# foollh/PicoPose

Measured on AMD Instinct MI355X. Metric: image-crops/sec (224x224, 162 templates), higher is better.
Workload: dtype f32 tensors; networks: f32 operands split into 2 f16 terms (22 bits) on f16 MFMA with f32 accumulate; stage-1 contraction: f16 MFMA operands, f32 accumulate, exact f32 re-evaluation of near-ties; PnP f64

## Files before the change

include/picopose_hip.h:

```cpp
#ifndef PICOPOSE_HIP_H
#define PICOPOSE_HIP_H

#include <stddef.h>
#include <stdint.h>

#ifdef __cplusplus
extern "C" {
#endif

#define PP_OK 0
#define PP_EINVAL (-1)
#define PP_EWORKSPACE (-2)
#define PP_ELAUNCH (-3)

#define PP_MATCH_EXACT 0
#define PP_MATCH_FAST 1

const char* pp_strerror(int code);
int pp_version(void);

int pp_prof_enable(int max_records);
int pp_prof_collect(float* out_ms, int max_out, int* count);
int pp_prof_gemm_enable(int max_records);
int pp_prof_gemm_collect(double* ms, double* flops, int* launches);
// ... 125 lines not shown
int pp_sum_slices(const float* part, int S, int M, int N, const float* bias, int act, float* out, void* stream);
int pp_hl_patch_columns(const float* x, int ld_x, int c, long long rows, void* hl, int ld_h, int col0, void* stream);

int pp_split_weights_t(const float* w, long long n, int terms, void* out, float* scale, void* stream);
int pp_split_activation_t(const float* x, long long batch_stride, int B, int P, int row_stride, int C, int relu, void* out,
                          int ld_h, int terms, void* stream);
int pp_hl_patch_columns_t(const float* x, int ld_x, int c, long long rows, void* out, int ld_h, int col0, int terms, void* stream);
int pp_layernorm_t(const float* x, const float* gamma, const float* beta, int rows, int C, float eps, float* y, void* out, int terms,
                   void* stream);
int pp_resize_bilinear_nhwc_t(const float* in, int B, int H, int W, int C, int Ho, int Wo, float mul, void* out, int terms,
                              void* stream);
int pp_resize_bilinear_nhwc_dual(const float* in, int B, int H, int W, int C, int Ho, int Wo, float mul, float* out, void* out_operand,
                                 int terms, void* stream);
int pp_warp_nhwc_t(const float* feat, int feat_batch, const float* flow, int B, int H, int W, int C, int ld_flow, void* out,
                   int ld_h, int terms, void* stream);
int pp_attention_t(const void* qkv_operand, int terms, int B, int T, int heads, int head_dim, float scale, float* out,
                   void* out_operand, void* stream);

int pp_attention(const float* qkv, int B, int T, int heads, int head_dim, float scale, float* out, void* stream);
int pp_attention_split(const float* qkv, int B, int T, int heads, int head_dim, float scale, float* out, void* out_hl,
                       void* stream);
int pp_attention_ex(const float* qkv, int B, int T, int heads, int head_dim, float scale, int prec, float* out, void* out_hl,
                    void* stream);
int pp_attention_hl(const void* qkv_hl, int B, int T, int heads, int head_dim, float scale, float* out, void* out_hl,
                    void* stream);
int pp_attention_train(const float* qkv, int B, int T, int heads, int head_dim, float scale, float* out, float* lse2, void* stream);
int pp_attention_backward(const float* qkv, const float* out, const float* dout, const float* lse2, const float* gpair, int B, int T,
                          int heads, int head_dim, float scale, float* Dws, float* dqkv, void* stream);

int pp_layernorm(const float* x, const float* gamma, const float* beta, int rows, int C, float eps,
                 float* y, void* stream);
int pp_layernorm_split(const float* x, const float* gamma, const float* beta, int rows, int C, float eps, float* y,
                       void* hl, void* stream);
int pp_softmax_rows(float* x, int rows, int n, int ld, void* stream);
int pp_groupnorm_nhwc(const float* x, const float* gamma, const float* beta, int B, int HW, int C,
                      int groups, float eps, int relu, float* y, void* stream);
int pp_transpose_batched(const float* in, long long in_batch_stride, int B, int R, int C, float* out,
                         long long out_batch_stride, int ld_out, int col_off, void* stream);
int pp_assemble_tokens(const float* patches, const float* cls_token, const float* pos, int B, int T, int C,
                       float* tokens, void* stream);
int pp_normalize_rows(const float* x, int rows, int n, float eps, float* y, void* stream);

int pp_resize_bilinear_nhwc(const float* in, int B, int H, int W, int C, int Ho, int Wo, float mul,
                            float* out, void* stream);
int pp_resize_bilinear_nhwc_hl(const float* in, int B, int H, int W, int C, int Ho, int Wo, float mul, void* out_hl,
                               void* stream);
int pp_warp_nhwc(const float* feat, int feat_batch, const float* flow, int B, int H, int W, int C, int ld_flow,
                 float* out, int ld_out, void* stream);
int pp_warp_nhwc_hl(const float* feat, int feat_batch, const float* flow, int B, int H, int W, int C, int ld_flow,
                    void* out_hl, int ld_h, void* stream);
int pp_avgpool2_nhwc(const float* in, int B, int H, int W, int C, float* out, void* stream);
int pp_gather_rows(const float* src, const long long* index, long long n_src_rows, long long row_floats, int n, float* dst,
                   void* stream);

int pp_crop_resize_normalize(const unsigned char* image, int H, int W, const unsigned char* mask, int y1, int y2, int x1,
                             int x2, int S, int rgb_mask_flag, const double* mean3, const double* std3, float* out_rgb,
                             float* out_mask, void* stream);
int pp_depth_points_nearest(const float* depth_m, int H, int W, int y1, int y2, int x1, int x2, int P, float fx, float fy,
                            float cx, float cy, float* out_pts, void* stream);
int pp_corr_lookup_nhwc(const float* f1, int ld_f1, const float* f2_l0, const float* f2_l1, const float* f2_l2,
                        int f2_batch, const float* flow, int B, int H, int W, int C, int levels, int radius,
                        int ld_flow, float* out, int ld_out, void* stream);
int pp_corr_lookup_nhwc_ex(const float* f1, int ld_f1, const float* f2_l0, const float* f2_l1, const float* f2_l2,
                           int f2_batch, const float* flow, int B, int H, int W, int C, int levels, int radius,
                           int ld_flow, int prec, float* out, int ld_out, void* stream);

int pp_conv_narrow_hl(const void* x_hl, int ld_x, int B, int H, int W, int C, const float* weight, const float* bias, int ksize,
                      int n_out, const float* residual, float* out, void* stream);
int pp_conv_narrow_f32(const float* x, int ld_x, int B, int H, int W, int C, const float* weight, const float* bias, int ksize,
                       int n_out, const float* residual, float* out, void* stream);

int pp_winograd_input_f32(const float* x, int ld_x, long long batch_stride, int B, int H, int W, int C, int relu, float* U, void* stream);
int pp_winograd_weight_f32(const float* w, int Cout, int Cin, int ldw, float* V, void* stream);
int pp_winograd_output_f32(const float* Y, int B, int H, int W, int Cout, const float* bias, int act, const float* residual,
                           const float* residual2, float* out, int ldc, void* stream);

int pp_winograd4_input_hl(const void* x_hl, int ld_x, long long batch_stride, int B, int H, int W, int C, int relu, void* U_hl, long long P_pad,
                          void* stream);
int pp_winograd4_weight_f32(const float* w, int Cout, int Cin, int ldw, float* V, void* stream);
int pp_winograd4_output(const float* Y, int ld_y, int B, int H, int W, int Cout, const float* bias, int act, const float* residual,
                        const float* residual2, float* out, int ldc, void* out_hl, int ld_h, int c_relu, long long P_pad, void* stream);

int pp_winograd4_chain(const float* Y, int ld_y, int B, int H, int W, int C, const float* bias, int act, int c_relu, void* U_hl, long long P_pad,
                       void* stream);

int pp_winograd_chain_f32(const float* Y, int B, int H, int W, int C, const float* bias, int act, int relu_next, float* U, void* stream);

int pp_set_saturation_word(unsigned int* word);

int pp_saturation_take(unsigned int* word, unsigned int* slot, void* stream);


int pp_corr_lookup_nhwc_hl(const void* f1_hl, int ld_f1, const void* f2_hl_l0, const void* f2_hl_l1, const void* f2_hl_l2,
                           int f2_batch, const float* flow, int B, int H, int W, int C, int levels, int radius, int ld_flow,
                           float* out, int ld_out, void* stream);

int pp_pnp_ransac(const float* tar_pts_2d, const float* src_pts_3d, const float* K, const float* tem_pose,
                  const int64_t* tar_pts, const int64_t* src_pts, int P, int H, int W, int N, int iterations,
                  float reproj_threshold, double* rot, double* tvec, double* inlier_ratio, int32_t* success,
                  int32_t* num_points, void* stream);

int pp_pnp_ransac_debug(const float* tar_pts_2d, const float* src_pts_3d, const float* K, const float* tem_pose,
                        const int64_t* tar_pts, const int64_t* src_pts, int P, int H, int W, int N, int iterations,
                        float reproj_threshold, double* rot, double* tvec, double* inlier_ratio, int32_t* success,
                        int32_t* num_points, double* refit_branches, void* stream);

// ... 240 lines not shown
```

picopose_amd/_lib.py:

```python
import ctypes
import os
import re

from .build import LIB

_HEADER = os.path.join(os.path.dirname(os.path.abspath(__file__)), "..", "include", "picopose_hip.h")

PP_OK = 0
PP_MATCH_EXACT = 0
PP_MATCH_FAST = 1
PP_BANK_F32 = 0
PP_BANK_F16 = 1

_lib = None


class PpGemmDesc(ctypes.Structure):
    _fields_ = [
        ("A", ctypes.c_void_p), ("B", ctypes.c_void_p), ("C", ctypes.c_void_p), ("bias", ctypes.c_void_p),
        ("gamma", ctypes.c_void_p), ("residual", ctypes.c_void_p), ("residual2", ctypes.c_void_p),
        ("M", ctypes.c_int), ("N", ctypes.c_int), ("K", ctypes.c_int),
        ("lda", ctypes.c_int), ("ldb", ctypes.c_int), ("ldc", ctypes.c_int), ("b_kn", ctypes.c_int),
        ("batch0", ctypes.c_int), ("batch1", ctypes.c_int),
        ("a_bs0", ctypes.c_longlong), ("a_bs1", ctypes.c_longlong), ("b_bs0", ctypes.c_longlong),
# ... 73 lines not shown
                                              vp, vp]
        L.pp_similarity_volume.argtypes = [vp, vp, vp, i32, i32, i32, i32, vp, vp]
        L.pp_calc_pred_Ms.argtypes = [vp, vp, vp, vp, vp, vp, i32, f32, vp, vp]
        L.pp_pose_recovery_2d.argtypes = [vp, vp, vp, vp, vp, vp, i32, vp, vp]
        L.pp_init_correspondences.argtypes = [vp, vp, i32, i32, i32, vp, vp, vp]
        L.pp_stage3_correspondences.argtypes = [vp, vp, i32, i32, i32, f32, vp, vp, vp]
        L.pp_gather_valid.argtypes = [vp, vp, i32, i32, i32, i32, i32, vp, vp, vp]
        L.pp_gemm.argtypes = [c.POINTER(PpGemmDesc), vp]
        L.pp_split_f16x3.argtypes = [vp, c.c_longlong, vp, vp, vp]
        L.pp_split_activation.argtypes = [vp, c.c_longlong, i32, i32, i32, i32, i32, vp, vp]
        L.pp_split_activation_ld.argtypes = [vp, c.c_longlong, i32, i32, i32, i32, i32, vp, i32, vp]
        L.pp_conv_narrow_hl.argtypes = [vp, i32, i32, i32, i32, i32, vp, vp, i32, i32, vp, vp, vp]
        L.pp_conv_narrow_f32.argtypes = [vp, i32, i32, i32, i32, i32, vp, vp, i32, i32, vp, vp, vp]
        L.pp_winograd_input_f32.argtypes = [vp, i32, c.c_longlong, i32, i32, i32, i32, i32, vp, vp]
        L.pp_winograd_weight_f32.argtypes = [vp, i32, i32, i32, vp, vp]
        L.pp_winograd_output_f32.argtypes = [vp, i32, i32, i32, i32, vp, i32, vp, vp, vp, i32, vp]
        L.pp_winograd4_input_hl.argtypes = [vp, i32, c.c_longlong, i32, i32, i32, i32, i32, vp, c.c_longlong, vp]
        L.pp_winograd4_weight_f32.argtypes = [vp, i32, i32, i32, vp, vp]
        L.pp_winograd4_output.argtypes = [vp, i32, i32, i32, i32, i32, vp, i32, vp, vp, vp, i32, vp, i32, i32, c.c_longlong, vp]
        L.pp_winograd4_chain.argtypes = [vp, i32, i32, i32, i32, i32, vp, i32, i32, vp, c.c_longlong, vp]
        L.pp_winograd_chain_f32.argtypes = [vp, i32, i32, i32, i32, vp, i32, i32, vp, vp]
        L.pp_set_saturation_word.argtypes = [vp]
        L.pp_saturation_take.argtypes = [vp, vp, vp]
        L.pp_split_weights_t.argtypes = [vp, c.c_longlong, i32, vp, vp, vp]
        L.pp_split_weights_ws.argtypes = [vp, c.c_longlong, i32, vp, vp, vp, vp]
        L.pp_split_activation_t.argtypes = [vp, c.c_longlong, i32, i32, i32, i32, i32, vp, i32, i32, vp]
        L.pp_hl_patch_columns_t.argtypes = [vp, i32, i32, c.c_longlong, vp, i32, i32, i32, vp]
        L.pp_layernorm_t.argtypes = [vp, vp, vp, i32, i32, f32, vp, vp, i32, vp]
        L.pp_resize_bilinear_nhwc_t.argtypes = [vp, i32, i32, i32, i32, i32, i32, f32, vp, i32, vp]
        L.pp_resize_bilinear_nhwc_dual.argtypes = [vp, i32, i32, i32, i32, i32, i32, f32, vp, vp, i32, vp]
        L.pp_warp_nhwc_t.argtypes = [vp, i32, vp, i32, i32, i32, i32, i32, vp, i32, i32, vp]
        L.pp_attention_t.argtypes = [vp, i32, i32, i32, i32, i32, f32, vp, vp, vp]
        L.pp_sum_slices.argtypes = [vp, i32, i32, i32, vp, i32, vp, vp]
        L.pp_hl_patch_columns.argtypes = [vp, i32, i32, c.c_longlong, vp, i32, i32, vp]
        L.pp_warp_nhwc_hl.argtypes = [vp, i32, vp, i32, i32, i32, i32, i32, vp, i32, vp]
        L.pp_attention.argtypes = [vp, i32, i32, i32, i32, f32, vp, vp]
        L.pp_attention_split.argtypes = [vp, i32, i32, i32, i32, f32, vp, vp, vp]
        L.pp_attention_ex.argtypes = [vp, i32, i32, i32, i32, f32, i32, vp, vp, vp]
        L.pp_attention_hl.argtypes = [vp, i32, i32, i32, i32, f32, vp, vp, vp]
        L.pp_attention_train.argtypes = [vp, i32, i32, i32, i32, f32, vp, vp, vp]
        L.pp_attention_backward.argtypes = [vp, vp, vp, vp, vp, i32, i32, i32, i32, f32, vp, vp, vp]
        L.pp_layernorm.argtypes = [vp, vp, vp, i32, i32, f32, vp, vp]
        L.pp_layernorm_split.argtypes = [vp, vp, vp, i32, i32, f32, vp, vp, vp]
        L.pp_softmax_rows.argtypes = [vp, i32, i32, i32, vp]
        L.pp_groupnorm_nhwc.argtypes = [vp, vp, vp, i32, i32, i32, i32, f32, i32, vp, vp]
        L.pp_transpose_batched.argtypes = [vp, c.c_longlong, i32, i32, i32, vp, c.c_longlong, i32, i32, vp]
        L.pp_assemble_tokens.argtypes = [vp, vp, vp, i32, i32, i32, vp, vp]
        L.pp_normalize_rows.argtypes = [vp, i32, i32, f32, vp, vp]
        L.pp_resize_bilinear_nhwc.argtypes = [vp, i32, i32, i32, i32, i32, i32, f32, vp, vp]
        L.pp_resize_bilinear_nhwc_hl.argtypes = [vp, i32, i32, i32, i32, i32, i32, f32, vp, vp]
        L.pp_warp_nhwc.argtypes = [vp, i32, vp, i32, i32, i32, i32, i32, vp, i32, vp]
        L.pp_avgpool2_nhwc.argtypes = [vp, i32, i32, i32, i32, vp, vp]
        L.pp_gather_rows.argtypes = [vp, vp, c.c_longlong, c.c_longlong, i32, vp, vp]
        L.pp_depth_points_nearest.argtypes = [vp, i32, i32, i32, i32, i32, i32, i32, f32, f32, f32, f32, vp, vp]
        L.pp_crop_resize_normalize.argtypes = [vp, i32, i32, vp, i32, i32, i32, i32, i32, i32, c.POINTER(c.c_double),
                                               c.POINTER(c.c_double), vp, vp, vp]
        L.pp_corr_lookup_nhwc.argtypes = [vp, i32, vp, vp, vp, i32, vp, i32, i32, i32, i32, i32, i32, i32, vp, i32, vp]
        L.pp_corr_lookup_nhwc_ex.argtypes = [vp, i32, vp, vp, vp, i32, vp, i32, i32, i32, i32, i32, i32, i32, i32, vp, i32, vp]
        L.pp_corr_lookup_nhwc_hl.argtypes = [vp, i32, vp, vp, vp, i32, vp, i32, i32, i32, i32, i32, i32, i32, vp, i32, vp]
        L.pp_pnp_ransac.argtypes = [vp, vp, vp, vp, vp, vp, i32, i32, i32, i32, i32, f32, vp, vp, vp, vp, vp, vp]
        L.pp_pnp_ransac_debug.argtypes = [vp, vp, vp, vp, vp, vp, i32, i32, i32, i32, i32, f32, vp, vp, vp, vp, vp, vp, vp]
        L.pp_pnp_ransac_refine.argtypes = [vp, vp, vp, vp, vp, vp, i32, i32, i32, i32, i32, f32, i32, c.c_double] + [vp] * 10
        L.pp_pnp_refine_lm.argtypes = [vp] * 6 + [i32, i32, i32, c.c_double] + [vp] * 6
        L.pp_rgbd_ransac.argtypes = [vp] * 6 + [i32] * 4 + [vp, i32, i32, i32, vp, vp, i32] + [vp] * 9
        L.pp_train_keypoints_workspace_bytes.restype = sz
        L.pp_train_keypoints_workspace_bytes.argtypes = [i32]
        L.pp_train_keypoints.argtypes = [vp, vp, i32, i32, vp, vp, i32, i32] + [vp] * 10 + [i32, vp, vp, vp, sz, vp]
        L.pp_batchnorm_train_workspace_bytes.restype = sz
        L.pp_batchnorm_train_workspace_bytes.argtypes = [i32, i32]
        L.pp_batchnorm_train.argtypes = [vp, vp, vp, i32, i32, f32, f32, vp, vp, i32, vp, vp, vp, vp, sz, vp]
        L.pp_gather_normalize_rows.argtypes = [vp, c.c_longlong, vp, i32, i32, f32, vp, vp]
        L.pp_xent_diag_rows.argtypes = [vp, i32, i32, f32, vp, vp]
        L.pp_flow_loss_blocks.argtypes = []
        L.pp_flow_loss_sums.argtypes = [vp, vp, vp, i32, i32, i32, f32, vp, vp]
        ll = c.c_longlong
        L.pp_colsum_workspace_bytes.restype = sz
        L.pp_colsum_workspace_bytes.argtypes = [ll, i32]
        L.pp_colsum.argtypes = [vp, ll, i32, i32, vp, vp, sz, vp]
        L.pp_act_forward.argtypes = [vp, ll, i32, vp, vp]
        L.pp_act_backward.argtypes = [vp, vp, ll, i32, vp, vp]
        L.pp_elementwise.argtypes = [i32, vp, vp, ll, i32, vp, vp]
        L.pp_layernorm_backward.argtypes = [vp, vp, vp, i32, i32, f32, vp, vp, vp]
        L.pp_groupnorm_backward_nhwc.argtypes = [vp, vp, vp, vp, i32, i32, i32, i32, f32, i32, vp, vp, vp, vp]
        L.pp_softmax_backward_rows.argtypes = [vp, vp, ll, i32, vp, vp]
        L.pp_xent_diag_backward.argtypes = [vp, i32, i32, f32, vp, vp, vp]
        L.pp_normalize_rows_backward.argtypes = [vp, ll, vp, vp, i32, i32, f32, vp, vp]
        L.pp_scatter_add_rows.argtypes = [vp, vp, i32, i32, vp, vp]
        L.pp_im2col_nhwc.argtypes = [vp, i32, i32, i32, i32, i32, i32, i32, vp, vp]
        L.pp_col2im_nhwc.argtypes = [vp, i32, i32, i32, i32, i32, i32, i32, vp, vp]
        L.pp_simvol_backward.argtypes = [vp, vp, vp, i32, i32, i32, vp, vp]
        L.pp_im2col_t_nhwc.argtypes = [vp, i32, i32, i32, i32, i32, i32, i32, vp, vp]
        L.pp_pow2_scale.argtypes = [vp, ll, vp, vp]
        L.pp_pow2_scale_ws.argtypes = [vp, ll, vp, vp, vp]
        L.pp_split_scaled_t.argtypes = [vp, ll, i32, i32, vp, vp, i32, vp]
        L.pp_split_transpose_t.argtypes = [vp, ll, i32, i32, vp, vp, i32, vp]
        L.pp_split_transpose_ld.argtypes = [vp, ll, i32, i32, vp, vp, ll, i32, vp]
        L.pp_im2col_t_operand.argtypes = [vp, i32, i32, i32, i32, i32, i32, i32, vp, i32, vp]
        L.pp_split_with_scale_t.argtypes = [vp, ll, i32, vp, vp, vp]
        L.pp_batchnorm_train_backward_workspace_bytes.restype = sz
        L.pp_batchnorm_train_backward_workspace_bytes.argtypes = [ll, i32]
        L.pp_batchnorm_train_backward.argtypes = [vp, vp, vp, vp, ll, i32, f32, i32, vp, vp, vp, vp, sz, vp]
        L.pp_resize_bilinear_backward_nhwc.argtypes = [vp, i32, i32, i32, i32, i32, i32, f32, vp, vp]
        L.pp_avgpool2_backward_nhwc.argtypes = [vp, i32, i32, i32, i32, i32, vp, vp]
        L.pp_warp_backward_nhwc.argtypes = [vp, vp, vp, i32, i32, i32, i32, i32, vp, vp, vp]
        L.pp_corr_lookup_backward_nhwc.argtypes = [vp, vp, vp, vp, i32, i32, i32, i32, i32, i32, i32, i32, vp, vp, vp, vp]
        L.pp_warp_backward_nhwc_fixed.argtypes = [vp, vp, vp, i32, i32, i32, i32, i32, vp, vp, vp]
# ... 67 lines not shown
```

picopose_amd/csrc/pp_sample.hip:

```cpp

#include <hip/hip_runtime.h>
#include <stdlib.h>
#include <stdint.h>
#include "../../include/picopose_hip.h"
#include "pp_common.h"
#include "pp_crop_dev.h"

namespace {

typedef float f4 __attribute__((ext_vector_type(4)));

__device__ __forceinline__ float resize_blend(float a, float b, float c, float d, float hx, float lx, float hy, float ly, float mul) {
#pragma clang fp contract(off)
    const float top = fmaf(hx, a, lx * b), bot = fmaf(hx, c, lx * d);
    return (hy * top + ly * bot) * mul;
}

__global__ __launch_bounds__(256) void resize_kernel(const float* __restrict__ in, int H, int W, int C,
                                                     int Ho, int Wo, float mul, float* __restrict__ out,
                                                     _Float16* __restrict__ out_hl, int terms) {
    const int b = blockIdx.z, oy = blockIdx.y, tid = threadIdx.x;
    const float sy = Ho > 1 ? (float)(H - 1) / (float)(Ho - 1) : 0.f;
    const float sx = Wo > 1 ? (float)(W - 1) / (float)(Wo - 1) : 0.f;
    const float fy = sy * (float)oy;
// ... 379 lines not shown
                }
            };
            load_chunk(0, ra0, rb0);
            if (nk > 1) load_chunk(1, ra1, rb1);
            for (int kc = 0; kc < nk; kc += 2) {
                chunk(kc, ra0, rb0);
                if (kc + 1 < nk) chunk(kc + 1, ra1, rb1);
            }
            __syncthreads();
#pragma unroll
            for (int i = 0; i < 2; ++i)
#pragma unroll
                for (int j = 0; j < 2; ++j)
#pragma unroll
                    for (int e = 0; e < 16; ++e)
                        S[(i * 32 + (e >> 2) * 8 + lh * 4 + (e & 3)) * CSP + wv * 64 + j * 32 + l31] =
                            acc[i][j][e] * (EXACT ? inv_sqrt_c : inv_sqrt_c / (PP_A_SCALE * PP_A_SCALE));
            __syncthreads();
            for (int idx = tid; idx < CM * win * win; idx += 256) {
                const int m = idx / (win * win), o = idx - m * (win * win), ai = o / win, bi = o - ai * win;
                const int dx = s_bx[m] - ox, dy = s_by[m] - oy;
                if (s_state[m] == 0 && dx >= 0 && dx <= fit && dy >= 0 && dy <= fit) {
                    const float cx = s_cx[m], cy = s_cy[m];
                    const float wx1 = cx - floorf(cx), wy1 = cy - floorf(cy), wx0 = 1.f - wx1, wy0 = 1.f - wy1;
                    const float* t = S + m * CSP + (dy + bi) * CRW + dx + ai;
                    out[((size_t)b * H * W + (size_t)(y0 + (m >> 3)) * W + x0 + (m & 7)) * ld_out + l * win * win + o] =
                        t[0] * (wx0 * wy0) + t[1] * (wx1 * wy0) + t[CRW] * (wx0 * wy1) + t[CRW + 1] * (wx1 * wy1);
                }
            }
            __syncthreads();
            if (tid < CM && s_state[tid] == 0) {
                const int dx = s_bx[tid] - ox, dy = s_by[tid] - oy;
                if (dx >= 0 && dx <= fit && dy >= 0 && dy <= fit) {
                    s_state[tid] = 1;
                    atomicSub(&s_todo, 1);
                }
            }
            __syncthreads();
        }
        __syncthreads();
    }
}

__global__ __launch_bounds__(256) void gather_rows_kernel(const float* __restrict__ src, const long long* __restrict__ index,
                                                          long long row, long long nsrc, float* __restrict__ dst) {
    const long long r = index[blockIdx.y];
    if (r < 0 || r >= nsrc) return;
    const f4* s4 = (const f4*)(src + r * row);
    f4* d4 = (f4*)(dst + (long long)blockIdx.y * row);
    const long long n4 = row >> 2;
    for (long long i = (long long)blockIdx.x * 256 + threadIdx.x; i < n4; i += (long long)gridDim.x * 256) d4[i] = s4[i];
}

__global__ __launch_bounds__(64) void saturation_take_kernel(unsigned* __restrict__ word, unsigned* __restrict__ slot) {
    if (threadIdx.x == 0) *slot = atomicExch(word, 0u);
}

__global__ __launch_bounds__(256) void crop_resize_kernel(const unsigned char* __restrict__ img, int W,
                                                          const unsigned char* __restrict__ mask, int y1, int y2, int x1,
                                                          int x2, int S, int mask_rgb, double m0, double m1, double m2,
                                                          double s0, double s1, double s2, float* __restrict__ out_rgb,
                                                          float* __restrict__ out_mask) {
    const int i = blockIdx.x * 256 + threadIdx.x;
    if (i >= S * S) return;
    const int oy = i / S, ox = i - oy * S, h = y2 - y1, w = x2 - x1;
    int ya, yb, xa, xb;
    double fy, fx;
    pp_crop_taps(oy, h, S, ya, yb, fy);
    pp_crop_taps(ox, w, S, xa, xb, fx);
    const double mean[3] = {m0, m1, m2}, stdv[3] = {s0, s1, s2};
    auto px = [&](int yy, int xx, int c) -> double {
        const size_t p = (size_t)(y1 + yy) * W + (x1 + xx);
        double v = (double)img[p * 3 + (2 - c)] / 255.0;
        if (mask_rgb && mask && mask[p] == 0) v = 0.0;
        return v;
    };
#pragma unroll
    for (int c = 0; c < 3; ++c) out_rgb[(size_t)c * S * S + i] = pp_crop_blend(px, c, ya, yb, xa, xb, fx, fy, mean[c], stdv[c]);
    if (out_mask) {
        const int yi = pp_crop_nearest(oy, h, S), xi = pp_crop_nearest(ox, w, S);
        out_mask[i] = mask ? (float)mask[(size_t)(y1 + yi) * W + (x1 + xi)] : 1.f;
    }
}

__global__ __launch_bounds__(256) void depth_points_kernel(const float* __restrict__ depth, int W, int y1, int y2, int x1,
                                                           int x2, int P, float fx, float fy, float cx, float cy,
                                                           float* __restrict__ out) {
    const int i = blockIdx.x * 256 + threadIdx.x;
    if (i >= P * P) return;
    const int oy = i / P, ox = i - oy * P, h = y2 - y1, w = x2 - x1;
    const int y = y1 + pp_crop_nearest(oy, h, P), x = x1 + pp_crop_nearest(ox, w, P);
    pp_depth_point(depth[(size_t)y * W + x], x, y, fx, fy, cx, cy, out + 3 * i);
}


constexpr int NRW_PITCH = 144;

template <int KS, int NOUT, bool F32IN = false>
__global__ __launch_bounds__(256) void conv_narrow_kernel(const _Float16* __restrict__ x, int ldx, int H, int W, int C,
                                                          const float* __restrict__ w, const float* __restrict__ bias,
                                                          const float* __restrict__ residual, float* __restrict__ out) {
    constexpr int R = KS / 2;
    extern __shared__ __attribute__((aligned(16))) unsigned char nsm[];
    const int TH = 256 / W, bands = H / TH;
    const int b = blockIdx.x / bands, y0 = (blockIdx.x % bands) * TH;
    const int tid = threadIdx.x, ty = tid / W, tx = tid % W;
// ... 204 lines not shown
    if (ld_f1 < C || ld_f1 % 4 != 0 || ((uintptr_t)f1 % 16) != 0 || f2_batch <= 0) return PP_EINVAL;
    if (levels < 1 || levels > MAXL || radius < 1 || radius > MAXR) return PP_EINVAL;
    if ((levels > 1 && !f2_l1) || (levels > 2 && !f2_l2)) return PP_EINVAL;
    if ((H >> (levels - 1)) < 1 || (W >> (levels - 1)) < 1 || ld_flow < 2) return PP_EINVAL;
    const int win = 2 * radius + 1;
    if (ld_out < levels * win * win) return PP_EINVAL;
    const char* te = getenv("PP_CORR_TILED");
    const bool tiled = !(te && te[0] == '0');
    const bool aligned = (((uintptr_t)f2_l0 | (levels > 1 ? (uintptr_t)f2_l1 : 0) | (levels > 2 ? (uintptr_t)f2_l2 : 0)) % 16) == 0;
    if (tiled && H % CT == 0 && W % CT == 0 && C % CK == 0 && aligned)
        return corr_tiled_launch(false, f1, ld_f1, f2_l0, f2_l1, f2_l2, f2_batch, flow, B, H, W, C, levels, radius, ld_flow, out, ld_out, stream,
                                 prec == PP_PREC_F32, prec == PP_PREC_F16);
    const size_t smem = (size_t)4 * (C + MAXL * TW * TW) * sizeof(float);
    hipLaunchKernelGGL(corr_lookup_kernel, dim3((H * W + 3) / 4, B), dim3(256), smem, (hipStream_t)stream, f1, ld_f1,
                       f2_batch, f2_l0, f2_l1, f2_l2, flow, H, W, C, levels, radius, ld_flow, 1.0f / sqrtf((float)C), out,
                       ld_out);
    return pp_last_launch();
}

int pp_corr_lookup_nhwc_hl(const void* f1_hl, int ld_f1, const void* f2_hl_l0, const void* f2_hl_l1, const void* f2_hl_l2,
                           int f2_batch, const float* flow, int B, int H, int W, int C, int levels, int radius, int ld_flow,
                           float* out, int ld_out, void* stream) {
    if (!f1_hl || !f2_hl_l0 || !flow || !out || B <= 0 || H <= 0 || W <= 0 || C <= 0 || f2_batch <= 0) return PP_EINVAL;
    if (H % CT != 0 || W % CT != 0 || C % CK != 0 || ld_f1 < C || ld_f1 % 8 != 0) return PP_EINVAL;
    if (((uintptr_t)f1_hl | (uintptr_t)f2_hl_l0 | (uintptr_t)f2_hl_l1 | (uintptr_t)f2_hl_l2) % 16 != 0) return PP_EINVAL;
    if (levels < 1 || levels > MAXL || radius < 1 || radius > MAXR) return PP_EINVAL;
    if ((levels > 1 && !f2_hl_l1) || (levels > 2 && !f2_hl_l2)) return PP_EINVAL;
    if ((H >> (levels - 1)) < 1 || (W >> (levels - 1)) < 1 || ld_flow < 2) return PP_EINVAL;
    const int win = 2 * radius + 1;
    if (ld_out < levels * win * win) return PP_EINVAL;
    return corr_tiled_launch(true, f1_hl, ld_f1, f2_hl_l0, f2_hl_l1, f2_hl_l2, f2_batch, flow, B, H, W, C, levels, radius, ld_flow, out, ld_out,
                             stream);
}

int pp_corr_lookup_nhwc(const float* f1, int ld_f1, const float* f2_l0, const float* f2_l1, const float* f2_l2,
                        int f2_batch, const float* flow, int B, int H, int W, int C, int levels, int radius,
                        int ld_flow, float* out, int ld_out, void* stream) {
    return pp_corr_lookup_nhwc_ex(f1, ld_f1, f2_l0, f2_l1, f2_l2, f2_batch, flow, B, H, W, C, levels, radius, ld_flow,
                                  PP_PREC_F16X3, out, ld_out, stream);
}

int pp_gather_rows(const float* src, const long long* index, long long n_src_rows, long long row_floats, int n, float* dst,
                   void* stream) {
    if (!src || !index || !dst || n <= 0 || n_src_rows <= 0 || row_floats <= 0 || row_floats % 4 != 0 ||
        ((uintptr_t)src % 16) != 0 || ((uintptr_t)dst % 16) != 0)
        return PP_EINVAL;
    const long long n4 = row_floats / 4;
    const int gx = (int)((n4 + 255) / 256 < 64 ? (n4 + 255) / 256 : 64);
    hipLaunchKernelGGL(gather_rows_kernel, dim3(gx, n), dim3(256), 0, (hipStream_t)stream, src, index, row_floats, n_src_rows,
                       dst);
    return pp_last_launch();
}

int pp_saturation_take(unsigned int* word, unsigned int* slot, void* stream) {
    if (!word || !slot) return PP_EINVAL;
    hipLaunchKernelGGL(saturation_take_kernel, dim3(1), dim3(64), 0, (hipStream_t)stream, word, slot);
    return pp_last_launch();
}

int pp_crop_resize_normalize(const unsigned char* image, int H, int W, const unsigned char* mask, int y1, int y2, int x1,
                             int x2, int S, int rgb_mask_flag, const double* mean3, const double* std3, float* out_rgb,
                             float* out_mask, void* stream) {
    if (!image || !out_rgb || !mean3 || !std3 || H <= 0 || W <= 0 || S <= 0 || y1 < 0 || x1 < 0 || y2 > H || x2 > W ||
        y2 <= y1 || x2 <= x1)
        return PP_EINVAL;
    hipLaunchKernelGGL(crop_resize_kernel, dim3((S * S + 255) / 256), dim3(256), 0, (hipStream_t)stream, image, W, mask, y1, y2,
                       x1, x2, S, rgb_mask_flag, mean3[0], mean3[1], mean3[2], std3[0], std3[1], std3[2], out_rgb, out_mask);
    return pp_last_launch();
}

int pp_depth_points_nearest(const float* depth_m, int H, int W, int y1, int y2, int x1, int x2, int P, float fx, float fy,
                            float cx, float cy, float* out_pts, void* stream) {
    if (!depth_m || !out_pts || H <= 0 || W <= 0 || P <= 0 || y1 < 0 || x1 < 0 || y2 > H || x2 > W || y2 <= y1 || x2 <= x1 ||
        fx == 0.f || fy == 0.f)
        return PP_EINVAL;
    hipLaunchKernelGGL(depth_points_kernel, dim3((P * P + 255) / 256), dim3(256), 0, (hipStream_t)stream, depth_m, W, y1, y2, x1,
                       x2, P, fx, fy, cx, cy, out_pts);
    return pp_last_launch();
}

int pp_conv_narrow_hl(const void* x_hl, int ld_x, int B, int H, int W, int C, const float* weight, const float* bias, int ksize,
                      int n_out, const float* residual, float* out, void* stream) {
    if (!x_hl || !weight || !out || B <= 0 || H <= 0 || C <= 0 || C % 32 != 0 || ld_x < C || ld_x % 8 != 0) return PP_EINVAL;
    if ((W != 16 && W != 32 && W != 64) || H % (256 / W) != 0 || (ksize != 1 && ksize != 3) || (n_out != 1 && n_out != 2)) return PP_EINVAL;
    if (((uintptr_t)x_hl % 16) != 0) return PP_EINVAL;
    const int TH = 256 / W, R = ksize / 2;
    const size_t lds = (size_t)(TH + 2 * R) * (W + 2 * R) * NRW_PITCH;
    const dim3 grid((unsigned)(B * (H / TH)));
    hipStream_t st = (hipStream_t)stream;
#define NRW_LAUNCH(KS_, N_)                                                                                                        \
    hipLaunchKernelGGL((conv_narrow_kernel<KS_, N_>), grid, dim3(256), lds, st, (const _Float16*)x_hl, ld_x, H, W, C, weight, bias, \
                       residual, out)
    if (ksize == 3 && n_out == 2) NRW_LAUNCH(3, 2);
    else if (ksize == 3) NRW_LAUNCH(3, 1);
    else if (n_out == 2) NRW_LAUNCH(1, 2);
    else NRW_LAUNCH(1, 1);
#undef NRW_LAUNCH
    return pp_last_launch();
}

}
```

picopose_amd/model/stage1.py:

```python
import math

import torch
import torch.nn as nn
import torch.nn.functional as F

from .. import ops
from .common import Holder, Packed, conv_p, linear_p, norm_p

ARCH = {
    "vit_small": (384, 12, 6),
    "vit_base": (768, 12, 12),
    "vit_large": (1024, 24, 16),
    "vit_giant2": (1536, 40, 24),
}
DESCRIPTOR_MAP = {
    "dinov2_vits14": "vit_small",
    "dinov2_vitb14": "vit_base",
    "dinov2_vitl14": "vit_large",
    "dinov2_vitg14": "vit_giant2",
    "gigapose_dinov2": "vit_large",
}


def _block(dim):
# ... 40 lines not shown
        self.patch_size = self.dinov2.patch_size

    def _pos_embed(self, w0, h0):
        v = self.dinov2
        pos = v.pos_embed.float()
        N = pos.shape[1] - 1
        if w0 * h0 == N:
            return pos[0]
        sq = int(math.sqrt(N))
        sx, sy = float(w0 + v.interpolate_offset) / math.sqrt(N), float(h0 + v.interpolate_offset) / math.sqrt(N)
        grid = F.interpolate(pos[:, 1:].reshape(1, sq, sq, -1).permute(0, 3, 1, 2), scale_factor=(sx, sy),
                             mode="bicubic", antialias=False)
        assert grid.shape[-2] == w0 and grid.shape[-1] == h0
        return torch.cat([pos[0, :1], grid.permute(0, 2, 3, 1).reshape(w0 * h0, -1)], dim=0)

    def _pack(self):
        v = self.dinov2
        return {
            "patch_w": ops.pack_conv_weight(v.patch_embed.proj.weight.float(), cin_pad=8),
            "pos": {},
        }

    def _pos_wt(self, w0, h0):
        v = self.dinov2
        cache = self.__dict__.setdefault("_pos_wt_cache", {})
        key = (v.pos_embed.shape[1] - 1, w0, h0, str(v.pos_embed.device))
        pk = {"pos": cache}
        if key not in pk["pos"]:
            N = v.pos_embed.shape[1] - 1
            if w0 * h0 == N:
                pk["pos"][key] = None
            else:
                sq = int(math.sqrt(N))
                sx, sy = float(w0 + v.interpolate_offset) / math.sqrt(N), float(h0 + v.interpolate_offset) / math.sqrt(N)
                with torch.no_grad():
                    basis = torch.eye(N, dtype=torch.float32, device=v.pos_embed.device).reshape(1, N, sq, sq)
                    grid = F.interpolate(basis, scale_factor=(sx, sy), mode="bicubic", antialias=False)
                pk["pos"][key] = grid.reshape(N, w0 * h0).contiguous()
        return pk["pos"][key]

    def _pos(self, w0, h0):
        pk = self.packed()
        key = (w0, h0)
        if key not in pk["pos"]:
            with torch.no_grad():
                wt = self._pos_wt(w0, h0) if self.training else None
                if wt is not None:
                    pe = self.dinov2.pos_embed.float()[0]
                    pk["pos"][key] = torch.cat([pe[:1], wt.t() @ pe[1:]], dim=0).contiguous()
                else:
                    pk["pos"][key] = self._pos_embed(w0, h0).contiguous()
        return pk["pos"][key]

    def forward_tokens(self, x, last_block_fn=None, all_blocks=False, embed_fn=None, level_out=None):
        v = self.dinov2
        B, _, H, W = x.shape
        p = v.patch_size
        assert H % p == 0 and W % p == 0
        h0, w0 = H // p, W // p
        C, heads = v.embed_dim, v.num_heads
        hd = C // heads
        pk = self.packed()
        T = h0 * w0 + 1
        if embed_fn is not None:
            xs = embed_fn(self, x)
        else:
            img = ops.to_nhwc(x, c_pad=8)
            patches = ops.conv2d(img, pk["patch_w"], v.patch_embed.proj.bias, p, stride=p)
            tok = ops.assemble_tokens(patches.view(B, h0 * w0, C), v.cls_token.reshape(C), self._pos(h0, w0))
            xs = tok.view(B * T, C)
        outs = []
        for i, blk in enumerate(v.blocks):
            if last_block_fn is not None and (all_blocks or i == len(v.blocks) - 1):
                xs = last_block_fn(blk, xs, B, T, heads, hd)
                if i in self.blocks_to_take:
                    outs.append(xs.view(B, T, C))
                continue
            h = ops.layernorm(xs, blk.norm1.weight, blk.norm1.bias, 1e-6, out_split=True)
            qkv = ops.linear(h, blk.attn.qkv.weight, blk.attn.qkv.bias, out_split=True)
            o = ops.attention(qkv, B, T, heads, hd, out_split=True)
            xs = ops.linear(o, blk.attn.proj.weight, blk.attn.proj.bias, gamma=blk.ls1.gamma, residual=xs)
            h = ops.layernorm(xs, blk.norm2.weight, blk.norm2.bias, 1e-6, out_split=True)
            f = ops.linear(h, blk.mlp.fc1.weight, blk.mlp.fc1.bias, act="gelu", out_split=True)
            dst = None
            if level_out is not None and i in self.blocks_to_take:
                dst = level_out[0][self.blocks_to_take.index(i)][level_out[1] * T:(level_out[1] + B) * T]
            xs = ops.linear(f, blk.mlp.fc2.weight, blk.mlp.fc2.bias, gamma=blk.ls2.gamma, residual=xs, out=dst)
            if i in self.blocks_to_take:
                outs.append(xs.view(B, T, C))
        return outs, (h0, w0)

    def forward(self, x):
        with torch.no_grad():
            toks, (h0, w0) = self.forward_tokens(x)
            return [ops.tokens_to_nchw(t, 1, h0, w0) for t in toks]
```

picopose_amd/ops.py:

```python
import contextlib
import ctypes
import os
import threading

import torch

from . import _lib
from ._lib import PpGemmDesc

ACT = {None: 0, "none": 0, "relu": 1, "gelu": 2, "leaky01": 3, "tanh": 4}

PRECISION = "f16x3"
_PREC = {"f32": 0, "f16x3": 1, "f16": 2}
_split_cache = {}
_scope = threading.local()


def precision():
    return getattr(_scope, "mode", None) or PRECISION


def check_precision(mode):
    if mode is not None and mode not in _PREC:
        raise ValueError(f"unknown arithmetic mode {mode!r}: expected None or one of {sorted(_PREC)}")
# ... 1011 lines not shown
    if (f1_hl is not None and f2_hl is not None and precision() == "f16x3" and f2_hl.terms == 2 and H % 8 == 0 and W % 8 == 0 and C % 32 == 0
            and os.environ.get("PP_CORR_TILED", "1") != "0" and os.environ.get("PP_CORR_HL", "1") != "0"):
        tgt, col0 = f1_hl
        assert tgt.shape[0] == B * H * W and col0 % 8 == 0 and col0 + C <= tgt.shape[1] and f2_hl.shape == (f2.shape[0] * H * W, C)
        hls = [f2_hl.hl] + [split_activation(p, p.shape[0], p.shape[1] * p.shape[2], C, p.shape[1] * p.shape[2] * C, C) for p in pyr[1:]]
        _lib.check(_lib.lib().pp_corr_lookup_nhwc_hl(tgt.hl.data_ptr() + 4 * col0, tgt.shape[1], _p(hls[0]), _p(hls[1]) if levels > 1 else None,
                                                     _p(hls[2]) if levels > 2 else None, f2.shape[0], _p(flow), B, H, W, C, levels, radius,
                                                     flow.stride(2), _p(out), np_, _lib.stream_ptr()), "pp_corr_lookup_nhwc_hl")
        return out
    _lib.check(_lib.lib().pp_corr_lookup_nhwc_ex(_p(f1), f1.stride(2), _p(pyr[0]), _p(pyr[1]) if levels > 1 else None,
                                                 _p(pyr[2]) if levels > 2 else None, f2.shape[0], _p(flow), B, H, W, C,
                                                 levels, radius, flow.stride(2), 2 if precision() == "f16" else _fly_prec(), _p(out), np_,
                                                 _lib.stream_ptr()), "pp_corr_lookup_nhwc_ex")
    return out


def tokens_to_nchw(tokens, skip, H, W):
    B, T, C = tokens.shape
    assert tokens.is_contiguous()
    out = torch.empty(B, C, H, W, dtype=torch.float32, device=tokens.device)
    src = tokens[:, skip:]
    _lib.check(_lib.lib().pp_transpose_batched(_p(src), T * C, B, H * W, C, _p(out), 0, H * W, 0, _lib.stream_ptr()),
               "pp_transpose_batched")
    return out


def assemble_tokens(patches, cls_token, pos):
    B, T, C = patches.shape
    assert patches.is_contiguous() and pos.is_contiguous() and cls_token.is_contiguous()
    out = torch.empty(B, T + 1, C, dtype=torch.float32, device=patches.device)
    _lib.check(_lib.lib().pp_assemble_tokens(_p(patches), _p(cls_token), _p(pos), B, T, C, _p(out), _lib.stream_ptr()),
               "pp_assemble_tokens")
    return out


def normalize_rows(x, eps=1e-12):
    rows, n = x.shape
    assert x.is_contiguous()
    y = torch.empty_like(x)
    _lib.check(_lib.lib().pp_normalize_rows(_p(x), rows, n, float(eps), _p(y), _lib.stream_ptr()), "pp_normalize_rows")
    return y


def gather_rows(src, index):
    R = src.shape[0]
    row = src[0].numel()
    if row % 4 != 0 or not src.is_contiguous() or src.dtype != torch.float32 or src.data_ptr() % 16 != 0:
        return src[index]
    index = index.contiguous()
    dst = torch.empty((index.numel(),) + tuple(src.shape[1:]), dtype=torch.float32, device=src.device)
    _lib.check(_lib.lib().pp_gather_rows(_p(src), _p(index), R, row, index.numel(), _p(dst), _lib.stream_ptr()),
               "pp_gather_rows")
    return dst
```

picopose_amd/picopose.py:

```python
import os

import torch
import torch.nn as nn

from . import ops
from .model.stage1 import FeatureExtractor
from .model.stage2 import AffineRegressor
from .model.stage3 import OffsetRegressor
from .utils.augment import aug_gtM_noise
from .utils.correspondence import compute_init_correspondences, compute_stage3_correspondences
from .utils.keypoints import KeypointInput, KeyPointSampler
from .utils.loss_utils import compute_stage_two_loss, flow_level_losses, infonce_rows
from .utils.matching import matching_features_similarity, matching_templates, matching_templates_indexed
from .utils.pose_recovery import pose_recovery_2d_prediction
from .utils.torch_utils import calc_pred_Ms


BATCH_VIT_TRAIN = os.environ.get("PP_BATCH_VIT_TRAIN", "1") != "0"
BATCH_DPT = os.environ.get("PP_BATCH_DPT", "1") != "0"
PREFETCH_QUERY = os.environ.get("PP_PREFETCH_QUERY", "1") != "0"


def _tensor_key(t, fe=None):
    key = (t.data_ptr(), tuple(t.shape), t._version, ops.precision())
    return key if fe is None else key + (fe._signatures()[0],)


def _image_rows(p, b0, b1):
    q = p[b0:b1]
    hl = getattr(p, "_hl", None)
    if hl is not None:
        hw = p.shape[1] * p.shape[2]
        s = ops.Split(hl.hl[b0 * hw:b1 * hw], hl.terms)
        s.image = (b1 - b0, p.shape[1], p.shape[2])
        q._hl = s
    return q


class Net(nn.Module):
    def __init__(self, cfg):
        super().__init__()
        self.cfg = cfg
        self.keypoint_sampler = KeyPointSampler()
        self.feature_extractor = FeatureExtractor(cfg.stage1)
        self.affine_regressor = AffineRegressor(cfg.stage2)
        self.offset_regressor = OffsetRegressor(cfg.stage3)
        self.match_mode = None
        self.batch_hypotheses = True
        self.keep_stage3 = False
        self.last_stage3 = None
        self.train_backward = True
        self.precision = None
        self.range_fallbacks = 0

    @property
    def precision(self):
        return self._precision

    @precision.setter
    def precision(self, mode):
        self._precision = ops.check_precision(mode)

    def invalidate_packed(self):
        from .model.common import Packed

        for m in self.modules():
            if isinstance(m, Packed):
                m.invalidate_packed()
        self._query_stash = None

    def select_template_data(self, end_points, pred_id_src, k):
        idx = pred_id_src[:, k]
        rows = end_points.get("template_index")
        rows = torch.arange(idx.shape[0], device=idx.device) if rows is None else rows
        sel = {key: end_points[key][rows, idx] for key in ("tem_pose", "tem_K", "tem_M", "tem_mask", "tem_rgb", "tem_pts3d")}
        for key in ("real_pts2d", "real_K", "real_M", "real_mask", "real_pose"):
            sel[key] = end_points[key]
        return sel

    def precompute_templates(self, tem_rgb, chunk=54):
        fe, dpt = self.feature_extractor, self.offset_regressor.dpt_head
        feats, maps = [], [[], [], []]
        with torch.no_grad():
            for s0 in range(0, tem_rgb.shape[0], chunk):
                toks, (h0, w0) = fe.forward_tokens(tem_rgb[s0:s0 + chunk])
                feats.append(ops.tokens_to_nchw(toks[-1], 1, h0, w0))
                for k, m in enumerate(dpt.forward_nhwc([t[:, 1:].unflatten(1, (h0, w0)) for t in toks])):
                    maps[k].append(m)
        return {"feature": torch.cat(feats), "dpt": [torch.cat(m) for m in maps]}

    def forward_test_hyp(self, end_points, real, tem_cached=None):
        fe = self.feature_extractor
        real_tok, (h0, w0) = real[0], real[1]
        real_dpt = real[2] if len(real) > 2 else None
        levels = real[3] if len(real) > 3 else None
        output = {"tem_pose": end_points["tem_pose"]}
        output["tar_pts_2d"] = end_points["real_pts2d"].permute(0, 3, 2, 1)
        output["src_pts_3d"] = end_points["tem_pts3d"].permute(0, 3, 1, 2)
        pre = real[4] if len(real) > 4 else None
        if tem_cached is None and pre is not None and levels is not None:
            alloc, nxt = pre
            Bn, T = nxt.shape[0], h0 * w0 + 1
            both, _ = fe.forward_tokens(torch.cat([nxt, end_points["tem_rgb"]]), level_out=(alloc, 0))
            tem_tok = [t[Bn:] for t in both]
            self._query_stash = (_tensor_key(nxt, fe), [a[:Bn * T].clone() for a in alloc], (h0, w0), nxt)
            tem_last = ops.tokens_to_nchw(tem_tok[-1], 1, h0, w0)
        elif tem_cached is None:
            tem_tok, _ = fe.forward_tokens(end_points["tem_rgb"], level_out=None if levels is None else (levels, 0))
            tem_last = ops.tokens_to_nchw(tem_tok[-1], 1, h0, w0)
        else:
            tem_last, tem_dpt = tem_cached
        sim = matching_features_similarity(tem_last, ops.tokens_to_nchw(real_tok[-1], 1, h0, w0),
                                           end_points["tem_mask"], end_points["real_mask"])
        pred_translation, pred_scale, pred_inplane = self.affine_regressor(sim)
        pred_Ms = calc_pred_Ms(pred_scale, pred_inplane, pred_translation, end_points["tem_pose"], end_points["tem_K"],
                               end_points["tem_M"])
        output["pred_poses"] = pose_recovery_2d_prediction(end_points["real_M"], end_points["real_K"], pred_Ms,
                                                           end_points["tem_K"], end_points["tem_M"], end_points["tem_pose"])
        init_flow, init_certainty = compute_init_correspondences(pred_Ms, end_points["tem_mask"])
        as_img = lambda t: t[:, 1:].unflatten(1, (h0, w0))
        orr = self.offset_regressor
        if levels is not None and real_dpt is None and tem_cached is None:
            T = h0 * w0 + 1
            nT, nR = tem_tok[0].shape[0], levels[0].shape[0] // T - tem_tok[0].shape[0]
            both = orr.dpt_head.forward_nhwc([as_img(lv.view(-1, T, lv.shape[1])) for lv in levels])
            tem_dpt, real_dpt = [_image_rows(p_, 0, nT) for p_ in both], [_image_rows(p_, nT, nT + nR) for p_ in both]
        else:
            if real_dpt is None:
                real_dpt = orr.dpt_head.forward_nhwc([as_img(t) for t in real_tok])
            if tem_cached is None:
                tem_dpt = orr.dpt_head.forward_nhwc([as_img(t) for t in tem_tok])
        flows, certs = orr.flow_decoder.forward_nhwc(tem_dpt, real_dpt, ops.to_nhwc(init_flow), ops.to_nhwc(init_certainty))
        if self.keep_stage3:
            self.last_stage3 = (flows[-1], certs[-1])
        output["pred_tar_pts"], output["pred_src_pts"] = compute_stage3_correspondences(
            ops.to_nchw(flows[-1]), ops.to_nchw(certs[-1]), threshold=0.5)
        return output

    def forward_hypotheses(self, end_points, pred_id_src, real):
        hyp = pred_id_src.shape[1]
        cache = end_points.get("template_cache")
        tidx = end_points.get("template_index")

        def cached(rows, idx):
            if cache is None:
                return None
            obj = (cache["obj_index"] if tidx is None else tidx)[rows]
            return end_points["template_feature"][rows if tidx is None else obj, idx], [m[obj, idx] for m in cache["dpt"]]

        if not self.batch_hypotheses:
            rows = torch.arange(pred_id_src.shape[0], device=pred_id_src.device)
            return [self.forward_test_hyp(self.select_template_data(end_points, pred_id_src, k), real,
                                          cached(rows, pred_id_src[:, k])) for k in range(hyp)]
        real_tok, hw = real[0], real[1]
        real_dpt = real[2] if len(real) > 2 and real[2] is not None else None
        levels = real[3] if len(real) > 3 else None
        B = pred_id_src.shape[0]
        idx = pred_id_src.t().reshape(-1)
        rows = torch.arange(B, device=idx.device).repeat(hyp)
        rep = lambda t: t.repeat(hyp, *([1] * (t.dim() - 1)))
        N = end_points["tem_pose"].shape[1]
        trow = rows if tidx is None else tidx[rows]
        flat = trow * N + idx
        sel = {key: (ops.gather_rows(end_points[key].flatten(0, 1), flat) if end_points[key].is_contiguous()
                     else end_points[key][trow, idx])
               for key in ("tem_pose", "tem_K", "tem_M", "tem_mask", "tem_rgb", "tem_pts3d")}
        for key in ("real_pts2d", "real_K", "real_M", "real_mask", "real_pose"):
            sel[key] = rep(end_points[key])
        toks = ([rep(t) for t in real_tok] if real_dpt is None and levels is None
                else [None] * (len(real_tok) - 1) + [rep(real_tok[-1])])
        out = self.forward_test_hyp(sel, (toks, hw, real_dpt, levels if cache is None else None, real[4] if len(real) > 4 and cache is None else None),
                                    cached(rows, idx))
        return [{key: v[k * B:(k + 1) * B] for key, v in out.items()} for k in range(hyp)]

    TEMPLATE_KEYS = ("template_feature", "tem_pose", "tem_K", "tem_M", "tem_mask", "tem_rgb", "tem_pts3d")

    def _check_template_index(self, end_points):
        tidx = end_points["template_index"]
        B = end_points["real_rgb"].shape[0]
        if not isinstance(tidx, torch.Tensor) or tidx.dtype != torch.int64 or tuple(tidx.shape) != (B,) or tidx.device != end_points["real_rgb"].device:
            raise ValueError(f"template_index must be a ({B},) int64 tensor on the crops' device")
        lead = {key: tuple(end_points[key].shape[:2]) for key in self.TEMPLATE_KEYS if key in end_points}
        if len(set(lead.values())) != 1:
            raise ValueError(f"with template_index every template tensor is (O, N, ...) for the same O and N: {lead}")
        cache = end_points.get("template_cache")
        if cache is not None and cache["obj_index"] is not tidx and not torch.equal(cache["obj_index"].to(tidx.device), tidx):
            raise ValueError("template_cache['obj_index'] and template_index name different objects")

    def forward_test(self, end_points, hyp=5, next_real_rgb=None):
        with torch.no_grad():
            if "template_index" in end_points:
                self._check_template_index(end_points)
            fe = self.feature_extractor
            levels = None
            ops.saturation_word(end_points["real_rgb"].device)
            stash, self._query_stash = getattr(self, "_query_stash", None), None
            if BATCH_DPT and self.batch_hypotheses and end_points.get("template_cache") is None:
                B, _, H, W = end_points["real_rgb"].shape
                T = (H // fe.patch_size) * (W // fe.patch_size) + 1
                pre_ok = PREFETCH_QUERY and next_real_rgb is not None and tuple(next_real_rgb.shape[1:]) == (3, H, W) and next_real_rgb.is_contiguous()
                Bn = next_real_rgb.shape[0] if pre_ok else 0
                alloc = [torch.empty((Bn + (hyp + 1) * B) * T, fe.num_features, dtype=torch.float32, device=end_points["real_rgb"].device)
                         for _ in fe.blocks_to_take]
                levels = [a_[Bn * T:] for a_ in alloc]
                if stash is not None and stash[0] == _tensor_key(end_points["real_rgb"], fe) and stash[1][0].shape[0] == B * T:
                    (h0, w0) = stash[2]
                    for lv, st in zip(levels, stash[1]):
                        lv[hyp * B * T:].copy_(st)
                    real_tok = [lv[hyp * B * T:].view(B, T, -1) for lv in levels]
                else:
                    real_tok, (h0, w0) = fe.forward_tokens(end_points["real_rgb"], level_out=(levels, hyp * B))
                real = (real_tok, (h0, w0), None, levels, (alloc, next_real_rgb) if Bn else None)
            else:
                real_tok, (h0, w0) = fe.forward_tokens(end_points["real_rgb"])
                real_dpt = self.offset_regressor.dpt_head.forward_nhwc([t[:, 1:].unflatten(1, (h0, w0)) for t in real_tok])
                real = (real_tok, (h0, w0), real_dpt)
            query = ops.tokens_to_nchw(real_tok[-1], 1, h0, w0)
            if "template_index" in end_points:
                pred_score_src, pred_id_src = matching_templates_indexed(
# ... 81 lines not shown
```

Baseline: 522.1.

## Reuse template feature bank for last ViT level instead of recomputing final blocks

When precomputed template features exist, the ViT forward for template crops stops after the second-to-last tapped block. The last-level tokens are filled from the template feature bank by a new transpose-gather kernel, which skips the remaining transformer blocks for template images. It is on by default only in f16/f16x3 precision. The risk is that bank features computed at a different precision may differ slightly from a fresh forward pass.

Measured after the change: 570.8 (median of 6 runs). 1.09x the previous value.

```diff
diff --git a/include/picopose_hip.h b/include/picopose_hip.h
--- a/include/picopose_hip.h
+++ b/include/picopose_hip.h
@@ -201,6 +201,8 @@
 int pp_avgpool2_nhwc(const float* in, int B, int H, int W, int C, float* out, void* stream);
 int pp_gather_rows(const float* src, const long long* index, long long n_src_rows, long long row_floats, int n, float* dst,
                    void* stream);
+int pp_bank_rows_to_tokens(const float* bank, long long n_bank_rows, int C, int P, const long long* index, int n, float* tokens, int ld,
+                           int T, int skip, void* stream);
 
 int pp_crop_resize_normalize(const unsigned char* image, int H, int W, const unsigned char* mask, int y1, int y2, int x1,
                              int x2, int S, int rgb_mask_flag, const double* mean3, const double* std3, float* out_rgb,
diff --git a/picopose_amd/_lib.py b/picopose_amd/_lib.py
--- a/picopose_amd/_lib.py
+++ b/picopose_amd/_lib.py
@@ -149,6 +149,7 @@
         L.pp_warp_nhwc.argtypes = [vp, i32, vp, i32, i32, i32, i32, i32, vp, i32, vp]
         L.pp_avgpool2_nhwc.argtypes = [vp, i32, i32, i32, i32, vp, vp]
         L.pp_gather_rows.argtypes = [vp, vp, c.c_longlong, c.c_longlong, i32, vp, vp]
+        L.pp_bank_rows_to_tokens.argtypes = [vp, c.c_longlong, i32, i32, vp, i32, vp, i32, i32, i32, vp]
         L.pp_depth_points_nearest.argtypes = [vp, i32, i32, i32, i32, i32, i32, i32, f32, f32, f32, f32, vp, vp]
         L.pp_crop_resize_normalize.argtypes = [vp, i32, i32, vp, i32, i32, i32, i32, i32, i32, c.POINTER(c.c_double),
                                                c.POINTER(c.c_double), vp, vp, vp]
diff --git a/picopose_amd/csrc/pp_sample.hip b/picopose_amd/csrc/pp_sample.hip
--- a/picopose_amd/csrc/pp_sample.hip
+++ b/picopose_amd/csrc/pp_sample.hip
@@ -455,6 +455,31 @@
     for (long long i = (long long)blockIdx.x * 256 + threadIdx.x; i < n4; i += (long long)gridDim.x * 256) d4[i] = s4[i];
 }
 
+__global__ __launch_bounds__(256) void bank_rows_to_tokens_kernel(const float* __restrict__ bank, const long long* __restrict__ index,
+                                                                  long long nsrc, int C, int P, float* __restrict__ tokens, int ld, int T,
+                                                                  int skip) {
+    __shared__ float t[32][33];
+    const long long r = index[blockIdx.z];
+    if (r < 0 || r >= nsrc) return;
+    const int c0 = blockIdx.x * 32, p0 = blockIdx.y * 32;
+    const int tx = threadIdx.x & 31, ty = threadIdx.x >> 5;
+    const float* src = bank + (size_t)r * C * P;
+    float* dst = tokens + (size_t)blockIdx.z * T * ld;
+#pragma unroll
+    for (int i = 0; i < 4; ++i) {
+        const int c = c0 + ty + 8 * i, p = p0 + tx;
+        if (c < C && p < P) t[ty + 8 * i][tx] = src[(size_t)c * P + p];
+    }
+    __syncthreads();
+#pragma unroll
+    for (int i = 0; i < 4; ++i) {
+        const int p = p0 + ty + 8 * i, c = c0 + tx;
+        if (p < P && c < C) dst[(size_t)(skip + p) * ld + c] = t[tx][ty + 8 * i];
+    }
+    if (blockIdx.y == 0 && c0 + tx < C)
+        for (int s = ty; s < skip; s += 8) dst[(size_t)s * ld + c0 + tx] = 0.f;
+}
+
 __global__ __launch_bounds__(64) void saturation_take_kernel(unsigned* __restrict__ word, unsigned* __restrict__ slot) {
     if (threadIdx.x == 0) *slot = atomicExch(word, 0u);
 }
@@ -765,6 +790,17 @@
     return pp_last_launch();
 }
 
+int pp_bank_rows_to_tokens(const float* bank, long long n_bank_rows, int C, int P, const long long* index, int n, float* tokens, int ld,
+                           int T, int skip, void* stream) {
+    if (!bank || !index || !tokens || n_bank_rows <= 0 || C <= 0 || P <= 0 || n <= 0 || ld < C || skip < 0 || T <= 0 ||
+        (long long)skip + P > T)
+        return PP_EINVAL;
+    if (n > 65535 || (P + 31) / 32 > 65535) return PP_EINVAL;
+    hipLaunchKernelGGL(bank_rows_to_tokens_kernel, dim3((C + 31) / 32, (P + 31) / 32, n), dim3(256), 0, (hipStream_t)stream, bank, index,
+                       n_bank_rows, C, P, tokens, ld, T, skip);
+    return pp_last_launch();
+}
+
 int pp_saturation_take(unsigned int* word, unsigned int* slot, void* stream) {
     if (!word || !slot) return PP_EINVAL;
     hipLaunchKernelGGL(saturation_take_kernel, dim3(1), dim3(64), 0, (hipStream_t)stream, word, slot);
diff --git a/picopose_amd/model/stage1.py b/picopose_amd/model/stage1.py
--- a/picopose_amd/model/stage1.py
+++ b/picopose_amd/model/stage1.py
@@ -116,7 +116,7 @@
                     pk["pos"][key] = self._pos_embed(w0, h0).contiguous()
         return pk["pos"][key]
 
-    def forward_tokens(self, x, last_block_fn=None, all_blocks=False, embed_fn=None, level_out=None):
+    def forward_tokens(self, x, last_block_fn=None, all_blocks=False, embed_fn=None, level_out=None, full_depth=None):
         v = self.dinov2
         B, _, H, W = x.shape
         p = v.patch_size
@@ -134,7 +134,15 @@
             tok = ops.assemble_tokens(patches.view(B, h0 * w0, C), v.cls_token.reshape(C), self._pos(h0, w0))
             xs = tok.view(B * T, C)
         outs = []
+        if full_depth is not None:
+            assert last_block_fn is None and embed_fn is None, "full_depth is an inference shortcut: not under the training hooks"
+            assert len(self.blocks_to_take) >= 2 and 0 <= full_depth <= B
         for i, blk in enumerate(v.blocks):
+            if full_depth is not None and i == self.blocks_to_take[-2] + 1:
+                xs, B = xs[:full_depth * T], full_depth
+                if B == 0:
+                    outs.append(xs.view(0, T, C))
+                    break
             if last_block_fn is not None and (all_blocks or i == len(v.blocks) - 1):
                 xs = last_block_fn(blk, xs, B, T, heads, hd)
                 if i in self.blocks_to_take:
diff --git a/picopose_amd/ops.py b/picopose_amd/ops.py
--- a/picopose_amd/ops.py
+++ b/picopose_amd/ops.py
@@ -1087,3 +1087,16 @@
     _lib.check(_lib.lib().pp_gather_rows(_p(src), _p(index), R, row, index.numel(), _p(dst), _lib.stream_ptr()),
                "pp_gather_rows")
     return dst
+
+
+def bank_rows_to_tokens(bank, index, T, skip=1, out=None):
+    R, C = bank.shape[:2]
+    P = bank[0, 0].numel()
+    n = index.numel()
+    assert bank.is_contiguous() and bank.dtype == torch.float32 and index.dtype == torch.int64 and index.device == bank.device
+    if out is None:
+        out = torch.empty(n * T, C, dtype=torch.float32, device=bank.device)
+    assert out.dim() == 2 and out.dtype == torch.float32 and out.shape[0] == n * T and out.shape[1] >= C and out.stride(1) == 1 and out.device == bank.device
+    _lib.check(_lib.lib().pp_bank_rows_to_tokens(_p(bank), R, C, P, _p(index.contiguous()), n, _p(out), out.stride(0), T, skip,
+                                                 _lib.stream_ptr()), "pp_bank_rows_to_tokens")
+    return out
diff --git a/picopose_amd/picopose.py b/picopose_amd/picopose.py
--- a/picopose_amd/picopose.py
+++ b/picopose_amd/picopose.py
@@ -19,6 +19,7 @@
 BATCH_VIT_TRAIN = os.environ.get("PP_BATCH_VIT_TRAIN", "1") != "0"
 BATCH_DPT = os.environ.get("PP_BATCH_DPT", "1") != "0"
 PREFETCH_QUERY = os.environ.get("PP_PREFETCH_QUERY", "1") != "0"
+TEMPLATE_LAST_FROM_BANK = {"0": False, "1": True}.get(os.environ.get("PP_TEMPLATE_LAST_FROM_BANK"))
 
 
 def _tensor_key(t, fe=None):
@@ -51,6 +52,7 @@
         self.last_stage3 = None
         self.train_backward = True
         self.precision = None
+        self.template_last_from_bank = None
         self.range_fallbacks = 0
 
     @property
@@ -68,12 +70,27 @@
             if isinstance(m, Packed):
                 m.invalidate_packed()
         self._query_stash = None
+
+    def _last_from_bank(self, end_points):
+        on = self.template_last_from_bank
+        on = TEMPLATE_LAST_FROM_BANK if on is None else on
+        on = ops.precision() in ("f16x3", "f16") if on is None else on
+        bank = end_points.get("template_feature")
+        if not on or self.training or bank is None or end_points.get("template_cache") is not None:
+            return False
+        fe = self.feature_extractor
+        H, W = end_points["tem_rgb"].shape[-2:]
+        grid = (fe.num_features, H // fe.patch_size, W // fe.patch_size)
+        return (bank.dtype == torch.float32 and bank.dim() == 5 and tuple(bank.shape[2:]) == grid and bank.is_contiguous()
+                and tuple(bank.shape[:2]) == tuple(end_points["tem_rgb"].shape[:2]) and len(fe.blocks_to_take) >= 2)
 
     def select_template_data(self, end_points, pred_id_src, k):
         idx = pred_id_src[:, k]
         rows = end_points.get("template_index")
         rows = torch.arange(idx.shape[0], device=idx.device) if rows is None else rows
         sel = {key: end_points[key][rows, idx] for key in ("tem_pose", "tem_K", "tem_M", "tem_mask", "tem_rgb", "tem_pts3d")}
+        if self._last_from_bank(end_points):
+            sel["tem_bank"] = (end_points["template_feature"].flatten(0, 1), rows * end_points["template_feature"].shape[1] + idx)
         for key in ("real_pts2d", "real_K", "real_M", "real_mask", "real_pose"):
             sel[key] = end_points[key]
         return sel
@@ -98,18 +115,27 @@
         output["tar_pts_2d"] = end_points["real_pts2d"].permute(0, 3, 2, 1)
         output["src_pts_3d"] = end_points["tem_pts3d"].permute(0, 3, 1, 2)
         pre = real[4] if len(real) > 4 else None
+        bank = end_points.get("tem_bank") if tem_cached is None else None
+        T = h0 * w0 + 1
         if tem_cached is None and pre is not None and levels is not None:
             alloc, nxt = pre
-            Bn, T = nxt.shape[0], h0 * w0 + 1
-            both, _ = fe.forward_tokens(torch.cat([nxt, end_points["tem_rgb"]]), level_out=(alloc, 0))
+            Bn = nxt.shape[0]
+            both, _ = fe.forward_tokens(torch.cat([nxt, end_points["tem_rgb"]]), level_out=(alloc, 0), full_depth=None if bank is None else Bn)
             tem_tok = [t[Bn:] for t in both]
+            if bank is not None:
+                nT = tem_tok[0].shape[0]
+                tem_tok[-1] = ops.bank_rows_to_tokens(*bank, T, out=alloc[-1][Bn * T:(Bn + nT) * T]).view(nT, T, -1)
             self._query_stash = (_tensor_key(nxt, fe), [a[:Bn * T].clone() for a in alloc], (h0, w0), nxt)
-            tem_last = ops.tokens_to_nchw(tem_tok[-1], 1, h0, w0)
         elif tem_cached is None:
-            tem_tok, _ = fe.forward_tokens(end_points["tem_rgb"], level_out=None if levels is None else (levels, 0))
-            tem_last = ops.tokens_to_nchw(tem_tok[-1], 1, h0, w0)
+            tem_tok, _ = fe.forward_tokens(end_points["tem_rgb"], level_out=None if levels is None else (levels, 0),
+                                           full_depth=None if bank is None else 0)
+            if bank is not None:
+                nT = tem_tok[0].shape[0]
+                tem_tok[-1] = ops.bank_rows_to_tokens(*bank, T, out=None if levels is None else levels[-1][:nT * T]).view(nT, T, -1)
         else:
             tem_last, tem_dpt = tem_cached
+        if tem_cached is None:
+            tem_last = ops.tokens_to_nchw(tem_tok[-1], 1, h0, w0) if bank is None else ops.gather_rows(*bank)
         sim = matching_features_similarity(tem_last, ops.tokens_to_nchw(real_tok[-1], 1, h0, w0),
                                            end_points["tem_mask"], end_points["real_mask"])
         pred_translation, pred_scale, pred_inplane = self.affine_regressor(sim)
@@ -121,7 +147,6 @@
         as_img = lambda t: t[:, 1:].unflatten(1, (h0, w0))
         orr = self.offset_regressor
         if levels is not None and real_dpt is None and tem_cached is None:
-            T = h0 * w0 + 1
             nT, nR = tem_tok[0].shape[0], levels[0].shape[0] // T - tem_tok[0].shape[0]
             both = orr.dpt_head.forward_nhwc([as_img(lv.view(-1, T, lv.shape[1])) for lv in levels])
             tem_dpt, real_dpt = [_image_rows(p_, 0, nT) for p_ in both], [_image_rows(p_, nT, nT + nR) for p_ in both]
@@ -165,6 +190,8 @@
         sel = {key: (ops.gather_rows(end_points[key].flatten(0, 1), flat) if end_points[key].is_contiguous()
                      else end_points[key][trow, idx])
                for key in ("tem_pose", "tem_K", "tem_M", "tem_mask", "tem_rgb", "tem_pts3d")}
+        if self._last_from_bank(end_points):
+            sel["tem_bank"] = (end_points["template_feature"].flatten(0, 1), flat)
         for key in ("real_pts2d", "real_K", "real_M", "real_mask", "real_pose"):
             sel[key] = rep(end_points[key])
         toks = ([rep(t) for t in real_tok] if real_dpt is None and levels is None
```
